# jperezrua/mfas

Measured on AMD Instinct MI355X. Metric: candidate-archs trained/sec (NTU inner loop), higher is better.
Workload: dtype f32

## Files before the change

### mfas_amd/csrc/mfas_hip.hip

```cpp
#include <hip/hip_runtime.h>
#include <hip/hip_fp16.h>
#pragma clang fp contract(off)
#include <stdint.h>
#include <stdio.h>
#include <string.h>
#include <math.h>
#include <cmath>
#include <algorithm>
#include <string>
#include <vector>
#include <thread>
#include <chrono>
#include <dlfcn.h>

#include "mfas_hip.h"

#include "common.hip.h"
#include "sweep.hip.h"
#include "chain.hip.h"

struct StepArgs {
    SweepArgs sa;
    ChainArgs ca;
    int32_t nchain, _pad;
    GatherArgs ga;
};

template <int MB, bool NT, int WPE, bool LEAN, int NS = 1>
__global__ void __launch_bounds__(STEP_THREADS, WPE) k_step(const StepArgs a) {
    extern __shared__ __attribute__((aligned(16))) float lds[];
    const int bid = (int)blockIdx.x;
    if (bid < a.nchain) {
        if constexpr (NS > 1) {
            const int Kp = a.nchain / NS, part = bid / Kp, c = bid - part * Kp;
            if (c < a.ca.ncand) chain_split<NS>(a.ca, chain_step_of(a.ca), c, part, lds);
        } else
        if constexpr (LEAN) { chain_lean<MB, 0, (WPE >= 4 ? 8 : 16)>(a.ca, chain_step_of(a.ca), bid, lds, lean_pre<MB>(a.ca, bid)); chain_lean_tail<MB, 0>(a.ca, chain_step_of(a.ca), bid, lds); }
        else chain_body<MB, false>(a.ca, chain_step_of(a.ca), bid, lds);
    }
    else if (bid < a.nchain + a.ga.nblocks) gather_body(a.ga, a.ga.cands[bid - a.nchain], a.sa.g, a.sa.tab, a.sa.order, (int)threadIdx.x);
    else if (bid < a.nchain + a.ga.nblocks + a.sa.ntap) sweep_tap_body<MB, NT, SweepU<MB, WPE>::v>(a.sa, bid - a.nchain - a.ga.nblocks, lds);
    else sweep_body<MB, NT, SweepU<MB, WPE>::v, false, !LEAN>(a.sa, sweep_step_of(a.sa), bid - a.nchain - a.ga.nblocks - a.sa.ntap, lds);
}

template <int MB, bool NT, int NS = 1>
__global__ void __launch_bounds__(STEP_THREADS, 4) k_step_same(const StepArgs a) {
    extern __shared__ __attribute__((aligned(16))) float lds[];
    const int bid = (int)blockIdx.x;
    if (bid < a.nchain) {
        if constexpr (NS > 1) {
            const int Kp = a.nchain / NS, part = bid / Kp, c = bid - part * Kp;
            if (c < a.ca.ncand) chain_split<NS>(a.ca, chain_step_of(a.ca), c, part, lds);
        } else chain_body<MB, false, true>(a.ca, chain_step_of(a.ca), bid, lds);
    } else sweep_body<MB, NT, SweepU<MB, 4>::v, true>(a.sa, sweep_step_of(a.sa), bid - a.nchain, lds);
}

template <int MB, bool LEAN>
__global__ void __launch_bounds__(STEP_THREADS, 2) k_chain(const ChainArgs a) {
    extern __shared__ __attribute__((aligned(16))) float lds[];
    if constexpr (LEAN) { chain_lean<MB>(a, chain_step_of(a), (int)blockIdx.x, lds, lean_pre<MB>(a, (int)blockIdx.x)); chain_lean_tail<MB, 0>(a, chain_step_of(a), (int)blockIdx.x, lds); }
    else chain_body<MB, true>(a, chain_step_of(a), (int)blockIdx.x, lds);
}

#include "wide.hip.h"
#include "persist.hip.h"
#include "eval.hip.h"
#include "pack.hip.h"
#include "surrogate.hip.h"

#include "builds.hip.h"
#include "plan.hip.h"
#ifdef MFAS_TEST_HOOKS
#include "plan_dump.hip.h"
#endif

struct LaunchRecord {
    struct Entry { BuildKey key; const void* fn; int64_t n; };
    std::vector<Entry> entries;
    void clear() { entries.clear(); }
    void count(const BuildKey& key, const void* fn) {
        for (Entry& e : entries) if (e.fn == fn) { ++e.n; return; }
        entries.push_back(Entry{key, fn, 1});
    }
    std::string describe() const {
        std::vector<std::string> items;
        for (const Entry& e : entries) items.push_back(e.key.name() + ":" + std::to_string(e.n));
        std::sort(items.begin(), items.end());
        std::string out;
        for (const std::string& s : items) out += (out.empty() ? "" : " ") + s;
        return out;
    }
};

struct mfas_population {
    mfas_hyper hp;
    Tuning tune;
    int K = 0, device = 0, n_cus = 0;
    int chunk_cols_req = 0;
    hipStream_t stream = nullptr;
    LayoutPlan plan;
    float* plane = nullptr;
    float* wt = nullptr;
    float* stepbuf = nullptr;
    float* best = nullptr;
    CandDev* d_cands = nullptr;
    SegDesc* d_descs = nullptr;
    struct GroupDev { SegDesc* d_descs = nullptr; TapDesc* d_taps = nullptr; };
    std::vector<GroupDev> groups;
    DevStats* d_stats = nullptr;
    int32_t* d_status = nullptr;
    uint32_t* d_seeds = nullptr;
    long long* d_corr = nullptr;
    float* d_posw = nullptr;
    int stats_cap = 0;
    bool profiling = false;
    int prof_every = 16;
    std::vector<hipEvent_t> ev;
    int64_t prof_launches = 0;
    double prof_ms = 0.0, bytes_per_launch = 0.0, prof_bytes = 0.0;
    LaunchRecord launched;
    double best_threshold = 0.0;
    struct Progress {
        std::vector<int64_t> done, nb;
        std::vector<double> best_metric;
        std::vector<int32_t> keeps_best;
        void reset(int K, double threshold) { done.assign(K, 0); nb.assign(K, 0); best_metric.assign(K, threshold); keeps_best.assign(K, 0); }
    } prog;
    float* d_move = nullptr;
    int64_t move_cap = 0;
    uint32_t* d_red_cnt = nullptr;
    char* d_gather = nullptr;
    size_t gather_cap = 0;
    uint32_t* d_cellflag = nullptr;
    float* d_xch = nullptr;
    SegDesc* d_pdescs = nullptr;
    int fell_back = 0;
    uint32_t* d_sync = nullptr;
    int32_t* d_need = nullptr;
    int32_t* d_role = nullptr;
    float* d_scal = nullptr;
    size_t scal_cap = 0;
    unsigned long long* d_trace = nullptr;
    char* d_vote = nullptr;
    size_t vote_cap = 0;
};

namespace {
struct Roctx {
    int (*push)(const char*) = nullptr;
    int (*pop)() = nullptr;
    Roctx() {
        if (getenv("MFAS_NO_ROCTX")) return;
        void* h = dlopen("librocprofiler-sdk-roctx.so", RTLD_LAZY | RTLD_LOCAL);
        if (!h) h = dlopen("librocprofiler-sdk-roctx.so.1", RTLD_LAZY | RTLD_LOCAL);
        if (!h) h = dlopen("libroctx64.so", RTLD_LAZY | RTLD_LOCAL);
        if (!h) return;
        push = reinterpret_cast<int (*)(const char*)>(dlsym(h, "roctxRangePushA"));
        pop = reinterpret_cast<int (*)()>(dlsym(h, "roctxRangePop"));
        if (!push || !pop) { push = nullptr; pop = nullptr; }
    }
};
Roctx& roctx() { static Roctx r; return r; }
struct RangeGuard {
    bool on;
    explicit RangeGuard(const std::string& name) : on(roctx().push != nullptr) { if (on) roctx().push(name.c_str()); }
    ~RangeGuard() { if (on) roctx().pop(); }
};
}
extern "C" int mfas_range_push(const char* name) { if (name && roctx().push) roctx().push(name); return MFAS_OK; }
extern "C" int mfas_range_pop(void) { if (roctx().pop) roctx().pop(); return MFAS_OK; }

extern "C" const char* mfas_last_error(void) { return g_err.c_str(); }
extern "C" int mfas_version(void) { return 200; }
#ifndef MFAS_SRC_DIGEST
#define MFAS_SRC_DIGEST "unknown"
#endif
extern "C" const char* mfas_source_digest(void) { return "mfas-src-digest:" MFAS_SRC_DIGEST; }

template <typename KT>
static hipError_t set_lds(KT kernel, size_t bytes) {
    return hipFuncSetAttribute(reinterpret_cast<const void*>(kernel), hipFuncAttributeMaxDynamicSharedMemorySize, (int)bytes);
}

static_assert(BUILDS_NTR == PERSIST_NTR && BUILDS_NTR16 == PERSIST_NTR16 && BUILDS_DT_BF16 == MFAS_DT_BF16, "builds.hip.h restates these");
typedef void (*StepKernel)(const StepArgs);
typedef void (*ChainKernel)(const ChainArgs);
typedef void (*PresidentKernel)(const PersistArgs, const int);
typedef hipError_t (*EvalLaunch)(mfas_population*, const EvalArgs&, int, hipStream_t);

template <typename KT>
struct Build { BuildKey key; KT fn = nullptr; };
typedef Build<StepKernel> StepBuild;
typedef Build<ChainKernel> ChainBuild;
typedef Build<PresidentKernel> PresidentBuild;
typedef Build<EvalLaunch> EvalBuild;

template <int MBE, int NRBW, int MSP, bool XB, bool B3>
static hipError_t launch_eval_t(mfas_population* p, const EvalArgs& a, int ncand, hipStream_t st);

template <int MB, bool NT, int WPE, bool LEAN, int NS> static StepBuild step_of() { return {step_key_of(MB, NT, WPE, LEAN, NS), k_step<MB, NT, WPE, LEAN, NS>}; }
template <int MB, bool NT, int NS> static StepBuild same_of() { return {same_key_of(MB, NT, NS), k_step_same<MB, NT, NS>}; }
template <bool NT> static StepBuild wide_sweep_of() { return {sweep_wide_key_of(NT), k_sweep_wide<NT>}; }
template <int MB, bool LEAN> static ChainBuild chain_of() { return {chain_key_of(MB, LEAN), k_chain<MB, LEAN>}; }
template <int MB, int NTR, bool X16, int NU, int PLAIN> static PresidentBuild president_of() { return {president_key_of(MB, NTR, X16, NU, PLAIN), k_president<MB, NTR, X16, NU, PLAIN>}; }
template <int MBE, int NRBW, int MSP, bool XB, bool B3> static EvalBuild eval_of() { return {eval_key_of(MBE, NRBW, MSP, XB, B3), launch_eval_t<MBE, NRBW, MSP, XB, B3>}; }

template <typename KT, size_t N>
static Build<KT> find_build(const Build<KT> (&rows)[N], const BuildKey& key) {
    for (const Build<KT>& r : rows) if (r.key == key) return r;
    return Build<KT>();
}

static StepBuild step_build(const BuildKey& key) {
#define STEP_(...) step_of<__VA_ARGS__>(),
#define SAME_(...) same_of<__VA_ARGS__>(),
#define WIDE_(...) wide_sweep_of<__VA_ARGS__>(),
    static const StepBuild rows[] = {BUILDS_SAME_ROWS(SAME_) BUILDS_STEP_ROWS(STEP_) BUILDS_SWEEP_WIDE_ROWS(WIDE_)};
#undef STEP_
#undef SAME_
#undef WIDE_
    return find_build(rows, key);
}

static ChainBuild chain_build(const BuildKey& key) {
#define CHAIN_(...) chain_of<__VA_ARGS__>(),
    static const ChainBuild rows[] = {BUILDS_CHAIN_ROWS(CHAIN_) {chain_wide_key_of(), k_chain_wide}};
#undef CHAIN_
    return find_build(rows, key);
}

static PresidentBuild president_build(const BuildKey& key) {
#define PRES_(...) president_of<__VA_ARGS__>(),
    static const PresidentBuild rows[] = {BUILDS_PRESIDENT_ROWS(PRES_)};
#undef PRES_
    return find_build(rows, key);
}

static EvalBuild eval_build(const BuildKey& key) {
#define EVAL_(...) eval_of<__VA_ARGS__>(),
    static const EvalBuild rows[] = {BUILDS_EVAL_ROWS(EVAL_)};
#undef EVAL_
    return find_build(rows, key);
}

template <typename... A>
static void launch(void (*kernel)(A...), unsigned grid, size_t lds, hipStream_t stream, A... args) {
    void* argv[] = {const_cast<void*>(static_cast<const void*>(&args))...};
    (void)hipLaunchKernel(reinterpret_cast<const void*>(kernel), dim3(grid), dim3(STEP_THREADS), argv, lds, stream);
}

template <typename... A>
static void launch_build(mfas_population* p, const Build<void (*)(A...)>& b, unsigned grid, size_t lds, hipStream_t stream, A... args) {
    if (b.fn) p->launched.count(b.key, reinterpret_cast<const void*>(b.fn));
    launch(b.fn, grid, lds, stream, args...);
}

static hipError_t set_lds_all(const LayoutPlan& pl) {
    hipError_t e = hipSuccess;
    auto set = [&e](auto kernel, size_t bytes) { if (kernel && e == hipSuccess) e = set_lds(kernel, bytes); };
    for (const BuildKey& key : plan_keys(plan_facts(pl)))
        switch (key.family) {
            case F_STEP: set(step_build(key).fn, key.arg[4] > 1 ? pl.lds_split : pl.lds_step); break;
            case F_STEP_SAME: set(step_build(key).fn, key.arg[2] > 1 ? pl.lds_split : pl.lds_step); break;
            case F_SWEEP_WIDE: set(step_build(key).fn, pl.lds_step); break;
            case F_CHAIN: case F_CHAIN_WIDE: set(chain_build(key).fn, pl.lds_chain); break;
            case F_PRESIDENT: set(president_build(key).fn, pl.lds_president); break;
            default: break;
        }
    return e;
}

static int device_cus(int device) {
    int ncu = 0;
    if (hipDeviceGetAttribute(&ncu, hipDeviceAttributeMultiprocessorCount, device) != hipSuccess || ncu <= 0) ncu = 256;
    return ncu;
}

template <typename T>
static hipError_t upload(T** dst, const std::vector<T>& v) {
    if (v.empty()) return hipSuccess;
    hipError_t e = hipMalloc(dst, sizeof(T) * v.size());
    return e != hipSuccess ? e : hipMemcpy(*dst, v.data(), sizeof(T) * v.size(), hipMemcpyHostToDevice);
}

static int create_impl(const mfas_hyper* hp, const int32_t* confs, const int32_t* n_cells,
                       const uint32_t* drop_seeds, int32_t K, int32_t device, void* hip_stream,
                       int32_t chunk_cols, mfas_population** out, const bool allow_persist, const Tuning* inherit = nullptr) {
    if (!out) return fail(MFAS_EINVAL, "null argument or K <= 0");
    if (int vrc = validate_inputs(hp, confs, n_cells, K)) return vrc;
    hipError_t e = hipSetDevice(device);
    if (e != hipSuccess) return fail(MFAS_EHIP, std::string("hipSetDevice: ") + hipGetErrorString(e));
    mfas_population* p = new (std::nothrow) mfas_population();
    if (!p) return fail(MFAS_ENOMEM, "host alloc");
    p->hp = *hp;
    p->tune = inherit ? *inherit : tuning_from_env();
    p->K = K;
    p->device = device;
    p->stream = reinterpret_cast<hipStream_t>(hip_stream);
    p->chunk_cols_req = chunk_cols;
    p->n_cus = device_cus(device);
    p->prog.reset(K, 0.0);
    if (int prc = plan_layout(hp, confs, n_cells, drop_seeds, K, chunk_cols, p->n_cus, allow_persist, p->tune, p->plan)) { delete p; return prc; }
    const LayoutPlan& pl = p->plan;
    if (!pl.fits_lds) { delete p; return fail(MFAS_EINVAL, "geometry does not fit the 160 KiB LDS (R / batchsize too large)"); }
    p->bytes_per_launch = pl.bytes_per_launch;

#define CREATE_CHK(x)                                                                              \
    do {                                                                                           \
        hipError_t e_ = (x);                                                                       \
        if (e_ != hipSuccess) {                                                                    \
            std::string m_ = std::string(#x) + ": " + hipGetErrorString(e_);                       \
            mfas_population_destroy(p);                                                            \
            return fail(e_ == hipErrorOutOfMemory ? MFAS_ENOMEM : MFAS_EHIP, m_);                  \
        }                                                                                          \
    } while (0)
    const size_t wt_floats = (size_t)std::max<int64_t>(pl.wt_size, 64);
    CREATE_CHK(hipMalloc(&p->plane, sizeof(float) * 3 * (size_t)pl.plane_stride));
    CREATE_CHK(hipMalloc(&p->wt, sizeof(float) * wt_floats));
    CREATE_CHK(hipMalloc(&p->stepbuf, sizeof(float) * (size_t)pl.step_total));
    CREATE_CHK(hipMalloc(&p->d_status, sizeof(int32_t) * (K + 256)));
    CREATE_CHK(hipMemset(p->d_status, 0, sizeof(int32_t) * (K + 256)));
    CREATE_CHK(hipMalloc(&p->d_seeds, sizeof(uint32_t) * K));
    CREATE_CHK(hipMalloc(&p->d_corr, sizeof(long long)));
    CREATE_CHK(upload(&p->d_posw, std::vector<float>(pl.g.Cp, 1.0f)));
    CREATE_CHK(upload(&p->d_cands, pl.cands));
    CREATE_CHK(upload(&p->d_descs, pl.descs));
    p->groups.resize(pl.groups.size());
    for (size_t gi = 0; gi < pl.groups.size(); ++gi) {
        CREATE_CHK(upload(&p->groups[gi].d_descs, pl.groups[gi].descs));
        CREATE_CHK(upload(&p->groups[gi].d_taps, pl.groups[gi].taps));
    }
    if (pl.red_in_sweep) {
        CREATE_CHK(hipMalloc(&p->d_red_cnt, sizeof(uint32_t) * K * MFAS_MAX_CELLS));
        CREATE_CHK(hipMemset(p->d_red_cnt, 0, sizeof(uint32_t) * K * MFAS_MAX_CELLS));
    }
    if (pl.same_group) CREATE_CHK(hipMalloc(&p->d_cellflag, sizeof(uint32_t) * K * CELLFLAG_STRIDE));
    if (pl.chain_split) CREATE_CHK(hipMalloc(&p->d_xch, sizeof(float) * (size_t)K * XCH_CAND_FLOATS));
    CREATE_CHK(hipMemsetAsync(p->plane, 0, sizeof(float) * 3 * (size_t)pl.plane_stride, p->stream));
    CREATE_CHK(hipMemsetAsync(p->wt, 0, sizeof(float) * wt_floats, p->stream));
    CREATE_CHK(hipMemsetAsync(p->stepbuf, 0, sizeof(float) * (size_t)pl.step_total, p->stream));
    CREATE_CHK(set_lds_all(pl));
    if (pl.persist) {
        CREATE_CHK(upload(&p->d_pdescs, pl.pdescs));
        CREATE_CHK(upload(&p->d_need, pl.need));
        CREATE_CHK(upload(&p->d_role, pl.role));
// ... 297 lines not shown
```

### mfas_amd/csrc/sweep.hip.h

```cpp
#pragma once
#include "launches.hip.h"
template <int MB, bool NT, int SWEEP_U, bool COH = false, bool DBL = false>
__device__ __forceinline__ void tile_run(float* Wp, float* Mp, float* Vp, const int rb, const int nkb, const int kb0,
                                         const int kbs, const float* xt, const int ST, const float* xn, const int SN,
                                         const float (&dyf)[MB * 4], const float gsc, const AdamC& ac, const bool upd,
                                         const bool fwd, f32x4 (&yacc)[MB], float* T, const int tstride_rb,
                                         const int lane, const int nj, const bool store = true, const float* xp = nullptr,
                                         const float* dyp = nullptr, const float* dyc = nullptr, const int SDp = 0,
                                         const float ss_p = 0.f, const float bc2s_p = 1.f) {
    static_assert(!(DBL && COH), "the same-group launch defers nothing");
    const int l15 = lane & 15, lg = lane >> 4;
    const float a_ss = ac.ss, a_bc2s = ac.bc2s, a_w1 = ac.w1, a_b2 = ac.b2, a_w2 = ac.w2, a_eps = ac.eps, a_wd = ac.wd;
    for (int kbb = kb0; kbb < nkb; kbb += SWEEP_U * kbs) {
        f32x4 w4[SWEEP_U], m4[SWEEP_U], v4[SWEEP_U];
#pragma unroll
        for (int u = 0; u < SWEEP_U; ++u) {
            const int kb = kbb + u * kbs;
            if (kb < nkb) {
                const int64_t off = ((int64_t)rb * nkb + kb) * 256 + lane * 4;
                w4[u] = NT ? __builtin_nontemporal_load(reinterpret_cast<const f32x4*>(Wp + off))
                           : *reinterpret_cast<const f32x4*>(Wp + off);
                if (upd) {
                    m4[u] = NT ? __builtin_nontemporal_load(reinterpret_cast<const f32x4*>(Mp + off))
                               : *reinterpret_cast<const f32x4*>(Mp + off);
                    v4[u] = NT ? __builtin_nontemporal_load(reinterpret_cast<const f32x4*>(Vp + off))
                               : *reinterpret_cast<const f32x4*>(Vp + off);
                }
            }
        }
#pragma unroll
        for (int u = 0; u < SWEEP_U; ++u) {
            const int kb = kbb + u * kbs;
            if (kb < nkb) {
                const int64_t off = ((int64_t)rb * nkb + kb) * 256 + lane * 4;
                if (upd) {
                    int dq = lg * SDp + rb * 16 + l15;
                    if constexpr (DBL) asm volatile("" : "+v"(dq));
                    if constexpr (DBL) {
                        f32x4 accp = {0.f, 0.f, 0.f, 0.f};
                        DW_BATCH_LOOP(MB, nj, accp = MFMA16(xp[(4 * j + lg) * ST + kb * 16 + l15], dyp[dq + 4 * j * SDp], accp))
                        f32x4 w = w4[u], m = m4[u], v = v4[u];
                        adam4(w, m, v, accp * gsc, ss_p, bc2s_p, a_w1, a_b2, a_w2, a_eps, a_wd);
                        w4[u] = w; m4[u] = m; v4[u] = v;
                        __builtin_amdgcn_sched_barrier(0);
                    }
                    f32x4 acc = {0.f, 0.f, 0.f, 0.f};
                    if constexpr (DBL) { DW_BATCH_LOOP(MB, nj, acc = MFMA16(xt[(4 * j + lg) * ST + kb * 16 + l15], dyc[dq + 4 * j * SDp], acc)) }
                    else { DW_BATCH_LOOP(MB, (COH ? MB * 4 : nj), acc = MFMA16(xt[(4 * j + lg) * ST + kb * 16 + l15], dyf[j], acc)) }
                    { f32x4 w = w4[u], m = m4[u], v = v4[u];
                      adam4(w, m, v, acc * gsc, a_ss, a_bc2s, a_w1, a_b2, a_w2, a_eps, a_wd);
                      w4[u] = w; m4[u] = m; v4[u] = v; }
                    if (!COH && !DBL && !store) {
                    } else if (NT) {
                        __builtin_nontemporal_store(w4[u], reinterpret_cast<f32x4*>(Wp + off));
                        __builtin_nontemporal_store(m4[u], reinterpret_cast<f32x4*>(Mp + off));
                        __builtin_nontemporal_store(v4[u], reinterpret_cast<f32x4*>(Vp + off));
                    } else {
                        *reinterpret_cast<f32x4*>(Wp + off) = w4[u];
                        *reinterpret_cast<f32x4*>(Mp + off) = m4[u];
                        *reinterpret_cast<f32x4*>(Vp + off) = v4[u];
                    }
                    if (T) {
                        float* Tt = T + ((int64_t)kb * tstride_rb + rb) * 256;
                        const int base = (((l15 >> 2) * 16 + 4 * lg) << 2) + (l15 & 3);
#pragma unroll
                        for (int q = 0; q < 4; ++q) Tt[base + 4 * q] = w4[u][q];
                    }
                }
                if (fwd) {
#pragma unroll
                    for (int mb = 0; mb < MB; ++mb) {
                        const f32x4 x4 = *reinterpret_cast<const f32x4*>(xn + (mb * 16 + l15) * SN + kb * 16 + 4 * lg);
#pragma unroll
                        for (int q = 0; q < 4; ++q) yacc[mb] = MFMA16(x4[q], w4[u][q], yacc[mb]);
                    }
                }
            }
        }
    }
}

#define STEP_NW 8
#define STEP_THREADS (STEP_NW * 64)

struct SweepArgs {
    const SegDesc* desc;
    const TapDesc* tdesc;
    int32_t ntap, _padt;
    const CandDev* cands;
    float* plane;
    int64_t plane_stride;
    float* wt;
    float* stepbuf;
    mfas_table tab;
    const int32_t* order;
    int64_t pos_t, pos_n;
    int32_t base_t, base_n, nvalid_t, nvalid_n;
    int32_t do_update, do_forward;
    AdamC ac;
    Geo g;
    uint32_t* red_cnt;
    const uint32_t* cellflag;
    uint32_t flag_target;
    int32_t* flag_status;
    const char* gather;
    int64_t g_cand_stride, g_par_stride;
    int32_t g_par_t, g_par_n;
    int32_t mode, g_par_p;
    int64_t pos_p, sb_dy_prev;
    int32_t base_p, nvalid_p;
    float ss_p, bc2s_p;
};

__device__ __forceinline__ int64_t gather_tap_off(const Geo& g, const int kind, const int tap, const int eb) {
    int64_t o = 0;
#pragma unroll
    for (int u = 0; u < MFAS_MAX_TAPS; ++u) {
        if (kind == KIND_V || u < tap) o += g.sw[u];
        if (kind == KIND_V && u < tap) o += g.vw[u];
    }
    return o * g.Bp * eb;
}

struct GatherArgs {
    const CandDev* cands;
    char* buf;
    int64_t cand_stride, par_stride;
    int64_t pos[2];
    int32_t base[2], nvalid[2], par[2];
    int32_t nsets, nblocks;
};

__device__ __forceinline__ void gather_body(const GatherArgs& ga, const CandDev& cd, const Geo& g, const mfas_table& tab,
                                            const int32_t* order, const int tid) {
    const int eb = tab.dtype == MFAS_DT_F32 ? 4 : 2;
    const int32_t* ordp = cand_order(order, g, cd.gidx);
    uint32_t used = 0;
    for (int i = 0; i < cd.L; ++i) used |= (1u << cd.conf[i][0]) | (1u << (MFAS_MAX_TAPS + cd.conf[i][1]));
#pragma unroll
    for (int s = 0; s < 2; ++s) {
        if (s >= ga.nsets) break;
        char* dst0 = ga.buf + (int64_t)cd.gidx * ga.cand_stride + (int64_t)ga.par[s] * ga.par_stride;
        for (int kt = 0; kt < 2 * MFAS_MAX_TAPS; ++kt) {
            if (!((used >> kt) & 1u)) continue;
            const int kind = kt < MFAS_MAX_TAPS ? KIND_S : KIND_V, tap = kt & (MFAS_MAX_TAPS - 1);
            const int w = kind == KIND_S ? g.sw[tap] : g.vw[tap];
            const char* src0 = reinterpret_cast<const char*>(kind == KIND_S ? tab.s[tap] : tab.v[tap]);
            char* dst = dst0 + gather_tap_off(g, kind, tap, eb);
            const int vpr = (w * eb) >> 4, nvec = ga.nvalid[s] * vpr;
            for (int e0 = tid; e0 < nvec; e0 += 4 * STEP_THREADS) {
                u32x4 v[4];
#pragma unroll
                for (int u = 0; u < 4; ++u) {
                    const int e = e0 + u * STEP_THREADS;
                    if (e < nvec) {
                        const int b = e / vpr, c = e - b * vpr;
                        const int64_t row = ordp ? (int64_t)ordp[ga.pos[s] + b] : (int64_t)(ga.base[s] + b);
                        v[u] = *reinterpret_cast<const u32x4*>(src0 + (row * w) * eb + ((int64_t)c << 4));
                    }
                }
#pragma unroll
                for (int u = 0; u < 4; ++u) {
                    const int e = e0 + u * STEP_THREADS;
                    if (e < nvec) {
                        const int b = e / vpr, c = e - b * vpr;
                        *reinterpret_cast<u32x4*>(dst + ((int64_t)b * w) * eb + ((int64_t)c << 4)) = v[u];
                    }
                }
            }
        }
    }
}

struct SweepStep {
    int64_t pos_t, pos_n;
    int32_t base_t, base_n, nvalid_t, nvalid_n;
    int32_t upd, fwd;
    float ss, bc2s;
};
__device__ __forceinline__ SweepStep sweep_step_of(const SweepArgs& a) {
    SweepStep s;
    s.pos_t = a.pos_t; s.pos_n = a.pos_n; s.base_t = a.base_t; s.base_n = a.base_n;
    s.nvalid_t = a.nvalid_t; s.nvalid_n = a.nvalid_n; s.upd = a.do_update; s.fwd = a.do_forward;
    s.ss = a.ac.ss; s.bc2s = a.ac.bc2s;
    return s;
}


#ifdef MFAS_CHAIN_TIMING
#define SW_UNIT_STAMP(k) do { if (COH && a.cellflag && a.flag_target == 16u && threadIdx.x == 0 && d.cell == 0 && d.kind == KIND_S && d.k0 == 0 && d.cand == 0) a.flag_status[64 + 29 + (k)] = (int32_t)wall_clock64(); } while (0)
#define SW_END_STAMP() do { if (COH && a.cellflag && a.flag_target == 16u && threadIdx.x == 0) { atomicMax(reinterpret_cast<uint32_t*>(&a.flag_status[64 + 27]), (uint32_t)wall_clock64()); \
        atomicMax(reinterpret_cast<uint32_t*>(&a.flag_status[128 + d.cell * 4 + d.kind]), (uint32_t)wall_clock64()); } } while (0)
#else
#define SW_END_STAMP() do { } while (0)
#define SW_UNIT_STAMP(k) do { } while (0)
#endif
template <int MB, bool NT, int U, bool COH = false, bool DEFER = !COH>
__device__ __forceinline__ void sweep_body(const SweepArgs& a, const SweepStep& st, const int bid, float* lds) {
    const SegDesc d = a.desc[bid];
    const CandDev& cd = a.cands[d.cand];
    const int tid = threadIdx.x, lane = tid & 63, wave = tid >> 6;
    const int l15 = lane & 15, lg = lane >> 4;
    constexpr int Bp = MB * 16;
    const int cc = d.cc, rows_p = d.rows_p, nrb = rows_p >> 4, nkb = cc >> 4;
    const int ST = cc + 16;
    const int SN = cc + 4;
    const int SD = rows_p + 16;
    float* xt = lds;
    float* xn = xt + Bp * ST;
    float* dyl = xn + Bp * SN;
    const bool feat = d.kind <= KIND_V;
    const bool upd = st.upd != 0;
    const bool fwd = (st.fwd != 0) && feat;
    if (!upd && !fwd) return;
    float* wred = dyl + Bp * SD;
    const bool split_k = nrb < STEP_NW;
    const int mode = (DEFER && feat && upd) ? a.mode : LAUNCH_PLAIN;
    const bool dbl = mode == LAUNCH_DOUBLE;
    float* xp = wred + (split_k ? (nrb - 1) * STEP_NW * MB * 256 : 0);
    float* dyp = xp + Bp * ST;
    const int64_t sbo = cd.step_off;
    const bool red = a.red_cnt != nullptr;

    if (!COH && a.gather && feat) {
        const char* gb = a.gather + (int64_t)cd.gidx * a.g_cand_stride + gather_tap_off(a.g, d.kind, d.tap, a.tab.dtype == MFAS_DT_F32 ? 4 : 2);
        if (dbl) stage_table(xp, ST, gb + (int64_t)a.g_par_p * a.g_par_stride, a.tab.dtype, d.width, d.k0, cc, nullptr, 0, 0, a.nvalid_p, Bp, tid, STEP_THREADS);
        if (upd) stage_table(xt, ST, gb + (int64_t)a.g_par_t * a.g_par_stride, a.tab.dtype, d.width, d.k0, cc, nullptr, 0, 0, st.nvalid_t, Bp, tid, STEP_THREADS);
        if (fwd) stage_table(xn, SN, gb + (int64_t)a.g_par_n * a.g_par_stride, a.tab.dtype, d.width, d.k0, cc, nullptr, 0, 0, st.nvalid_n, Bp, tid, STEP_THREADS);
    } else {
    if (upd && feat) {
        const void* tp = d.kind == KIND_S ? a.tab.s[d.tap] : a.tab.v[d.tap];
        if (dbl) stage_table(xp, ST, tp, a.tab.dtype, d.width, d.k0, cc, cand_order(a.order, a.g, cd.gidx), a.pos_p, a.base_p, a.nvalid_p, Bp, tid, STEP_THREADS);
        stage_table(xt, ST, tp, a.tab.dtype, d.width, d.k0, cc, cand_order(a.order, a.g, cd.gidx), st.pos_t, st.base_t, st.nvalid_t, Bp, tid, STEP_THREADS);
    }
    if (fwd) {
        const void* tp = d.kind == KIND_S ? a.tab.s[d.tap] : a.tab.v[d.tap];
        stage_table(xn, SN, tp, a.tab.dtype, d.width, d.k0, cc, cand_order(a.order, a.g, cd.gidx), st.pos_n, st.base_n, st.nvalid_n, Bp, tid, STEP_THREADS);
    }
    }
    if constexpr (COH) {
        if (upd && a.cellflag) {
            __shared__ int s_go;
            if (tid == 0) {
                const int slot = d.kind == KIND_HEAD ? cd.L - 1 : (d.kind == KIND_OUT ? d.cell - 1 : d.cell);
                const uint32_t* f = a.cellflag + (size_t)cd.gidx * CELLFLAG_STRIDE + slot;
                uint32_t spins = 0;
                int go = 1;
                while (ld_u32_relaxed(f) < a.flag_target) {
                    __builtin_amdgcn_s_sleep(2);
                    if (++spins > CELLFLAG_SPIN_LIMIT) { go = 0; atomicMax(&a.flag_status[cd.gidx], 2); break; }
                }
                s_go = go;
#ifdef MFAS_CHAIN_TIMING
                if (a.flag_target == 16u && slot == 0 && d.kind <= KIND_V) atomicMin(reinterpret_cast<uint32_t*>(&a.flag_status[64 + 28]), (uint32_t)wall_clock64());
#endif
            }
            __syncthreads();
            if (!s_go) return;
            SW_UNIT_STAMP(0);
        }
    }
    if (upd) {
        if (!feat) {
            const int xcell = d.kind == KIND_OUT ? d.cell - 1 : cd.L - 1;
            stage_f32<COH>(xt, ST, a.stepbuf, sbo + a.g.sb_xo + (int64_t)xcell * Bp * a.g.Rp + d.k0, a.g.Rp, cc, Bp, tid, STEP_THREADS);
        }
        const int64_t dsrc = d.kind == KIND_HEAD ? sbo + a.g.sb_dlog : sbo + a.g.sb_dy + (int64_t)d.cell * Bp * a.g.Rp;
        stage_f32<COH>(dyl, SD, a.stepbuf, dsrc + d.rb0 * 16, d.seg_nrb * 16, rows_p, Bp, tid, STEP_THREADS);
        if (dbl) stage_f32<false>(dyp, SD, a.stepbuf, sbo + a.sb_dy_prev + (int64_t)d.cell * Bp * a.g.Rp + d.rb0 * 16, d.seg_nrb * 16, rows_p, Bp, tid, STEP_THREADS);
    }
    __syncthreads();
    SW_UNIT_STAMP(1);

    float* Wp = a.plane + d.w_off;
    float* Mp = Wp + a.plane_stride;
    float* Vp = Mp + a.plane_stride;
    const AdamC ac = adam_consts(a.ac, upd ? st.ss : 0.f, upd ? st.bc2s : 1.f);
    float gsc = 1.0f;
    if (a.g.alphas && feat && upd) gsc = ldc1<COH>(a.stepbuf + sbo + a.g.sb_gsc + d.cell * 2 + d.kind);

    const int rb0 = split_k ? 0 : wave, rbs = split_k ? 1 : STEP_NW;
    const int kb0 = split_k ? wave : 0, kbs = split_k ? STEP_NW : 1;
    const int64_t part = sbo + a.g.sb_part + (((int64_t)(cd.part_cell_off[d.cell] + d.part_idx) * d.seg_nrb * MB) << 8) +
                         (((int64_t)d.rb0 * MB) << 8);

    for (int rb = rb0; rb < nrb; rb += rbs) {
        float dyf[MB * 4];
        f32x4 yacc[MB];
#pragma unroll
        for (int mb = 0; mb < MB; ++mb) yacc[mb] = (f32x4){0.f, 0.f, 0.f, 0.f};
        float* Tt = d.wt_off >= 0 ? a.wt + d.wt_off + ((int64_t)(d.k0 >> 4) * d.seg_nrb + d.rb0) * 256 : nullptr;
        bool plain_walk = true;
        if constexpr (DEFER) {
            if (dbl) {
                plain_walk = false;
                tile_run<MB, NT, (U > 1 ? U / 2 : 1), false, true>(Wp, Mp, Vp, rb, nkb, kb0, kbs, xt, ST, xn, SN, dyf, gsc, ac, upd, fwd, yacc, Tt, d.seg_nrb,
                                                                    lane, (a.g.B + 3) >> 2, true, xp, dyp, dyl, SD, a.ss_p, a.bc2s_p);
                if (split_k && fwd && rb == nrb - 1) __syncthreads();
            }
        }
        if (plain_walk) {
#pragma unroll
            for (int j = 0; j < MB * 4; ++j) dyf[j] = upd ? dyl[(4 * j + lg) * SD + rb * 16 + l15] : 0.f;
            tile_run<MB, NT, U, COH>(Wp, Mp, Vp, rb, nkb, kb0, kbs, xt, ST, xn, SN, dyf, gsc, ac, upd, fwd, yacc, Tt, d.seg_nrb, lane,
                                     (a.g.B + 3) >> 2, mode != LAUNCH_VIRTUAL);
        }
        if (fwd) {
#pragma unroll
            for (int mb = 0; mb < MB; ++mb) {
                if (split_k)
                    *reinterpret_cast<f32x4*>(wred + (((rb * STEP_NW + wave) * MB + mb) << 8) + lane * 4) = yacc[mb];
                else if (red) stc4<true>(a.stepbuf, part + ((rb * MB + mb) << 8) + lane * 4, yacc[mb]);
                else
                    stc4<COH>(a.stepbuf, part + ((rb * MB + mb) << 8) + lane * 4, yacc[mb]);
            }
        }
    }
    SW_UNIT_STAMP(2);
    if (!fwd) { SW_END_STAMP(); return; }
    if (split_k) {
        __syncthreads();
        for (int e = tid; e < nrb * MB * 64; e += STEP_THREADS) {
            const int slot = e >> 6, ln = e & 63;
            const int srb = slot / MB, smb = slot - srb * MB;
            f32x4 s = *reinterpret_cast<const f32x4*>(wred + (((srb * STEP_NW) * MB + smb) << 8) + ln * 4);
#pragma unroll
            for (int w = 1; w < STEP_NW; ++w)
                s += *reinterpret_cast<const f32x4*>(wred + (((srb * STEP_NW + w) * MB + smb) << 8) + ln * 4);
            if (red) stc4<true>(a.stepbuf, part + (slot << 8) + ln * 4, s);
            else stc4<COH>(a.stepbuf, part + (slot << 8) + ln * 4, s);
        }
    }
    if (!red) { SW_END_STAMP(); return; }
    asm volatile("s_waitcnt vmcnt(0)" ::: "memory");
    __syncthreads();
    SW_UNIT_STAMP(3);
    int* flagw = reinterpret_cast<int*>(lds);
    const int ns_c = cd.nch_s[d.cell], nch_c = ns_c + cd.nch_v[d.cell];
    if (tid == 0) {
        uint32_t* cnt = a.red_cnt + d.cand * MFAS_MAX_CELLS + d.cell;
        const uint32_t old = __hip_atomic_fetch_add(cnt, 1u, __ATOMIC_RELAXED, __HIP_MEMORY_SCOPE_AGENT);
        const int last = old == (uint32_t)(nch_c - 1);
        if (last) __hip_atomic_store(cnt, 0u, __ATOMIC_RELAXED, __HIP_MEMORY_SCOPE_AGENT);
        flagw[0] = last;
    }
    __syncthreads();
    SW_UNIT_STAMP(4);
    if (!flagw[0]) { SW_END_STAMP(); return; }
    {
        const int snrb = d.seg_nrb;
        const int per_cell = snrb * MB * 64;
        const int64_t part0 = sbo + a.g.sb_part + (((int64_t)cd.part_cell_off[d.cell] * snrb * MB) << 8);
        const int64_t yf0 = sbo + a.g.sb_yf + (int64_t)d.cell * per_cell * 4;
        const int64_t vplane = (int64_t)MFAS_MAX_CELLS * snrb * MB * 256;
        for (int it = tid; it < per_cell; it += STEP_THREADS) {
            f32x4 accS = {0.f, 0.f, 0.f, 0.f}, accV = {0.f, 0.f, 0.f, 0.f};
            constexpr int PB = 8;
            for (int ch0 = 0; ch0 < nch_c; ch0 += PB) {
                f32x4 p8[PB];
#pragma unroll
                for (int u = 0; u < PB; ++u)
                    if (ch0 + u < nch_c) p8[u] = ldc4<true>(a.stepbuf, part0 + (((int64_t)(ch0 + u) * snrb * MB) << 8) + it * 4);
#pragma unroll
                for (int u = 0; u < PB; ++u)
                    if (ch0 + u < nch_c) {
                        if (ch0 + u < ns_c) accS += p8[u]; else accV += p8[u];
                    }
            }
            if (a.g.alphas) {
                *reinterpret_cast<f32x4*>(a.stepbuf + yf0 + it * 4) = accS;
                *reinterpret_cast<f32x4*>(a.stepbuf + yf0 + vplane + it * 4) = accV;
            } else {
                *reinterpret_cast<f32x4*>(a.stepbuf + yf0 + it * 4) = accS + accV;
            }
        }
    }
    SW_END_STAMP();
}

template <int MB, bool NT, int U>
__device__ __forceinline__ void sweep_tap_body(const SweepArgs& a, const int bid, float* lds) {
    const TapDesc& d = a.tdesc[bid];
    const int tid = threadIdx.x, lane = tid & 63, wave = tid >> 6;
    const int l15 = lane & 15, lg = lane >> 4;
    constexpr int Bp = MB * 16;
    const int cc = d.cc, rows_p = d.rows_p, nrb = rows_p >> 4, nkb = cc >> 4;
    const int ST = cc + 16, SN = cc + 4;
    float* xt = lds;
    float* xn = xt + Bp * ST;
    const bool upd = a.do_update != 0;
    const bool fwd = a.do_forward != 0;
    if (!upd && !fwd) return;
    const void* tp = d.kind == KIND_S ? a.tab.s[d.tap] : a.tab.v[d.tap];
    if (upd) stage_table(xt, ST, tp, a.tab.dtype, d.width, d.k0, cc, a.order, a.pos_t, a.base_t, a.nvalid_t, Bp, tid, STEP_THREADS);
    if (fwd) stage_table(xn, SN, tp, a.tab.dtype, d.width, d.k0, cc, a.order, a.pos_n, a.base_n, a.nvalid_n, Bp, tid, STEP_THREADS);
    __syncthreads();
    const int item = wave / nrb, rb = wave - item * nrb;
    if (item >= d.nitems) return;
    const CandDev& cd = a.cands[d.cand[item]];
    float* sb = a.stepbuf + cd.step_off;
    const int cell = d.cell[item];
    float dyf[MB * 4];
#pragma unroll
    for (int j = 0; j < MB * 4; ++j) dyf[j] = 0.f;
    if (upd) {
        const float* dsrc = sb + a.g.sb_dy + (int64_t)cell * Bp * a.g.Rp;
#pragma unroll
        for (int j = 0; j < MB * 4; ++j) dyf[j] = dsrc[(4 * j + lg) * rows_p + rb * 16 + l15];
    }
    float gsc = 1.0f;
    if (a.g.alphas && upd) gsc = sb[a.g.sb_gsc + cell * 2 + d.kind];
    float* Wp = a.plane + d.w_off[item];
    float* Mp = Wp + a.plane_stride;
    float* Vp = Mp + a.plane_stride;
    const AdamC ac = adam_consts(a.ac, a.ac.ss, a.ac.bc2s);
    f32x4 yacc[MB];
#pragma unroll
    for (int mb = 0; mb < MB; ++mb) yacc[mb] = (f32x4){0.f, 0.f, 0.f, 0.f};
    tile_run<MB, NT, U>(Wp, Mp, Vp, rb, nkb, 0, 1, xt, ST, xn, SN, dyf, gsc, ac, upd, fwd, yacc, nullptr, nrb, lane, (a.g.B + 3) >> 2);
    if (fwd) {
        float* part = sb + a.g.sb_part + (((int64_t)(cd.part_cell_off[cell] + d.part_idx[item]) * nrb * MB) << 8);
#pragma unroll
        for (int mb = 0; mb < MB; ++mb)
            *reinterpret_cast<f32x4*>(part + ((rb * MB + mb) << 8) + lane * 4) = yacc[mb];
    }
}
```

Before: 37.29.

## Add software-pipelined double-buffered sweep tile loop for MB=1, WPE=4 fused step

Factors the sweep tile body (load, dW MFMA plus Adam update, store, forward MFMA) into helpers. It adds a new tile_pipe path that double-buffers the W/M/V loads, issuing the next tile's loads before processing the current one, with sched barriers to keep that order. The path also makes wave and loop indices scalar via readfirstlane. It is enabled only for the k_step sweep when MB==1, WPE==4 and not LEAN, and only for feature segments doing both update and forward without a transposed copy. The aim is to hide global-memory latency in the optimizer sweep, at the cost of more registers and a second code path that must stay consistent with tile_run.

New measurement: 39.06, median of 6. +4.7%, better.

```diff
diff --git a/mfas_amd/csrc/mfas_hip.hip b/mfas_amd/csrc/mfas_hip.hip
--- a/mfas_amd/csrc/mfas_hip.hip
+++ b/mfas_amd/csrc/mfas_hip.hip
@@ -40,7 +40,7 @@
     }
     else if (bid < a.nchain + a.ga.nblocks) gather_body(a.ga, a.ga.cands[bid - a.nchain], a.sa.g, a.sa.tab, a.sa.order, (int)threadIdx.x);
     else if (bid < a.nchain + a.ga.nblocks + a.sa.ntap) sweep_tap_body<MB, NT, SweepU<MB, WPE>::v>(a.sa, bid - a.nchain - a.ga.nblocks, lds);
-    else sweep_body<MB, NT, SweepU<MB, WPE>::v, false, !LEAN>(a.sa, sweep_step_of(a.sa), bid - a.nchain - a.ga.nblocks - a.sa.ntap, lds);
+    else sweep_body<MB, NT, SweepU<MB, WPE>::v, false, !LEAN, SweepPipe<MB, WPE, LEAN>::v>(a.sa, sweep_step_of(a.sa), bid - a.nchain - a.ga.nblocks - a.sa.ntap, lds);
 }
 
 template <int MB, bool NT, int NS = 1>
diff --git a/mfas_amd/csrc/sweep.hip.h b/mfas_amd/csrc/sweep.hip.h
--- a/mfas_amd/csrc/sweep.hip.h
+++ b/mfas_amd/csrc/sweep.hip.h
@@ -1,5 +1,63 @@
 #pragma once
 #include "launches.hip.h"
+template <bool NT>
+__device__ __forceinline__ f32x4 tile_ld(const float* p) {
+    return NT ? __builtin_nontemporal_load(reinterpret_cast<const f32x4*>(p)) : *reinterpret_cast<const f32x4*>(p);
+}
+template <int MB, bool COH>
+__device__ __forceinline__ void tile_update(f32x4& w, f32x4& m, f32x4& v, const float* xt, const int ST, const int kb,
+                                            const float (&dyf)[MB * 4], const int nj, const int l15, const int lg, const float gsc,
+                                            const float ss, const float bc2s, const float w1, const float b2, const float w2,
+                                            const float eps, const float wd) {
+    f32x4 acc = {0.f, 0.f, 0.f, 0.f};
+    DW_BATCH_LOOP(MB, (COH ? MB * 4 : nj), acc = MFMA16(xt[(4 * j + lg) * ST + kb * 16 + l15], dyf[j], acc))
+    adam4(w, m, v, acc * gsc, ss, bc2s, w1, b2, w2, eps, wd);
+}
+template <int MB>
+__device__ __forceinline__ void tile_update_lds(f32x4& w, f32x4& m, f32x4& v, const float* x, const int ST, const int kb,
+                                                const float* dy, const int dq, const int SD, const int nj, const int l15, const int lg,
+                                                const float gsc, const float ss, const float bc2s, const float w1, const float b2,
+                                                const float w2, const float eps, const float wd) {
+    f32x4 acc = {0.f, 0.f, 0.f, 0.f};
+    DW_BATCH_LOOP(MB, nj, acc = MFMA16(x[(4 * j + lg) * ST + kb * 16 + l15], dy[dq + 4 * j * SD], acc))
+    adam4(w, m, v, acc * gsc, ss, bc2s, w1, b2, w2, eps, wd);
+}
+template <int MB>
+__device__ __forceinline__ void tile_replay(f32x4& w, f32x4& m, f32x4& v, const float* xp, const int ST, const int kb, const float* dyp,
+                                            const int dq, const int SD, const int nj, const int l15, const int lg, const float gsc,
+                                            const float ss_p, const float bc2s_p, const float w1, const float b2, const float w2,
+                                            const float eps, const float wd) {
+    tile_update_lds<MB>(w, m, v, xp, ST, kb, dyp, dq, SD, nj, l15, lg, gsc, ss_p, bc2s_p, w1, b2, w2, eps, wd);
+    __builtin_amdgcn_sched_barrier(0);
+}
+template <bool NT>
+__device__ __forceinline__ void tile_store(const f32x4 w, const f32x4 m, const f32x4 v, float* Wp, float* Mp, float* Vp, const int64_t off) {
+    if (NT) {
+        __builtin_nontemporal_store(w, reinterpret_cast<f32x4*>(Wp + off));
+        __builtin_nontemporal_store(m, reinterpret_cast<f32x4*>(Mp + off));
+        __builtin_nontemporal_store(v, reinterpret_cast<f32x4*>(Vp + off));
+    } else {
+        *reinterpret_cast<f32x4*>(Wp + off) = w;
+        *reinterpret_cast<f32x4*>(Mp + off) = m;
+        *reinterpret_cast<f32x4*>(Vp + off) = v;
+    }
+}
+__device__ __forceinline__ void tile_store_t(const f32x4 w, float* T, const int kb, const int tstride_rb, const int rb, const int l15, const int lg) {
+    float* Tt = T + ((int64_t)kb * tstride_rb + rb) * 256;
+    const int base = (((l15 >> 2) * 16 + 4 * lg) << 2) + (l15 & 3);
+#pragma unroll
+    for (int q = 0; q < 4; ++q) Tt[base + 4 * q] = w[q];
+}
+template <int MB>
+__device__ __forceinline__ void tile_forward(f32x4 (&yacc)[MB], const float* xn, const int SN, const int kb, const int l15, const int lg, const f32x4 w) {
+#pragma unroll
+    for (int mb = 0; mb < MB; ++mb) {
+        const f32x4 x4 = *reinterpret_cast<const f32x4*>(xn + (mb * 16 + l15) * SN + kb * 16 + 4 * lg);
+#pragma unroll
+        for (int q = 0; q < 4; ++q) yacc[mb] = MFMA16(x4[q], w[q], yacc[mb]);
+    }
+}
+
 template <int MB, bool NT, int SWEEP_U, bool COH = false, bool DBL = false>
 __device__ __forceinline__ void tile_run(float* Wp, float* Mp, float* Vp, const int rb, const int nkb, const int kb0,
                                          const int kbs, const float* xt, const int ST, const float* xn, const int SN,
@@ -18,13 +76,10 @@
             const int kb = kbb + u * kbs;
             if (kb < nkb) {
                 const int64_t off = ((int64_t)rb * nkb + kb) * 256 + lane * 4;
-                w4[u] = NT ? __builtin_nontemporal_load(reinterpret_cast<const f32x4*>(Wp + off))
-                           : *reinterpret_cast<const f32x4*>(Wp + off);
+                w4[u] = tile_ld<NT>(Wp + off);
                 if (upd) {
-                    m4[u] = NT ? __builtin_nontemporal_load(reinterpret_cast<const f32x4*>(Mp + off))
-                               : *reinterpret_cast<const f32x4*>(Mp + off);
-                    v4[u] = NT ? __builtin_nontemporal_load(reinterpret_cast<const f32x4*>(Vp + off))
-                               : *reinterpret_cast<const f32x4*>(Vp + off);
+                    m4[u] = tile_ld<NT>(Mp + off);
+                    v4[u] = tile_ld<NT>(Vp + off);
                 }
             }
         }
@@ -34,49 +89,86 @@
             if (kb < nkb) {
                 const int64_t off = ((int64_t)rb * nkb + kb) * 256 + lane * 4;
                 if (upd) {
-                    int dq = lg * SDp + rb * 16 + l15;
-                    if constexpr (DBL) asm volatile("" : "+v"(dq));
                     if constexpr (DBL) {
-                        f32x4 accp = {0.f, 0.f, 0.f, 0.f};
-                        DW_BATCH_LOOP(MB, nj, accp = MFMA16(xp[(4 * j + lg) * ST + kb * 16 + l15], dyp[dq + 4 * j * SDp], accp))
-                        f32x4 w = w4[u], m = m4[u], v = v4[u];
-                        adam4(w, m, v, accp * gsc, ss_p, bc2s_p, a_w1, a_b2, a_w2, a_eps, a_wd);
-                        w4[u] = w; m4[u] = m; v4[u] = v;
-                        __builtin_amdgcn_sched_barrier(0);
+                        int dq = lg * SDp + rb * 16 + l15;
+                        asm volatile("" : "+v"(dq));
+                        tile_replay<MB>(w4[u], m4[u], v4[u], xp, ST, kb, dyp, dq, SDp, nj, l15, lg, gsc, ss_p, bc2s_p, a_w1, a_b2, a_w2, a_eps, a_wd);
+                        tile_update_lds<MB>(w4[u], m4[u], v4[u], xt, ST, kb, dyc, dq, SDp, nj, l15, lg, gsc, a_ss, a_bc2s, a_w1, a_b2, a_w2, a_eps, a_wd);
+                    } else {
+                        tile_update<MB, COH>(w4[u], m4[u], v4[u], xt, ST, kb, dyf, nj, l15, lg, gsc, a_ss, a_bc2s, a_w1, a_b2, a_w2, a_eps, a_wd);
                     }
-                    f32x4 acc = {0.f, 0.f, 0.f, 0.f};
-                    if constexpr (DBL) { DW_BATCH_LOOP(MB, nj, acc = MFMA16(xt[(4 * j + lg) * ST + kb * 16 + l15], dyc[dq + 4 * j * SDp], acc)) }
-                    else { DW_BATCH_LOOP(MB, (COH ? MB * 4 : nj), acc = MFMA16(xt[(4 * j + lg) * ST + kb * 16 + l15], dyf[j], acc)) }
-                    { f32x4 w = w4[u], m = m4[u], v = v4[u];
-                      adam4(w, m, v, acc * gsc, a_ss, a_bc2s, a_w1, a_b2, a_w2, a_eps, a_wd);
-                      w4[u] = w; m4[u] = m; v4[u] = v; }
                     if (!COH && !DBL && !store) {
-                    } else if (NT) {
-                        __builtin_nontemporal_store(w4[u], reinterpret_cast<f32x4*>(Wp + off));
-                        __builtin_nontemporal_store(m4[u], reinterpret_cast<f32x4*>(Mp + off));
-                        __builtin_nontemporal_store(v4[u], reinterpret_cast<f32x4*>(Vp + off));
                     } else {
-                        *reinterpret_cast<f32x4*>(Wp + off) = w4[u];
-                        *reinterpret_cast<f32x4*>(Mp + off) = m4[u];
-                        *reinterpret_cast<f32x4*>(Vp + off) = v4[u];
+                        tile_store<NT>(w4[u], m4[u], v4[u], Wp, Mp, Vp, off);
                     }
-                    if (T) {
-                        float* Tt = T + ((int64_t)kb * tstride_rb + rb) * 256;
-                        const int base = (((l15 >> 2) * 16 + 4 * lg) << 2) + (l15 & 3);
-#pragma unroll
-                        for (int q = 0; q < 4; ++q) Tt[base + 4 * q] = w4[u][q];
-                    }
+                    if (T) tile_store_t(w4[u], T, kb, tstride_rb, rb, l15, lg);
                 }
-                if (fwd) {
-#pragma unroll
-                    for (int mb = 0; mb < MB; ++mb) {
-                        const f32x4 x4 = *reinterpret_cast<const f32x4*>(xn + (mb * 16 + l15) * SN + kb * 16 + 4 * lg);
-#pragma unroll
-                        for (int q = 0; q < 4; ++q) yacc[mb] = MFMA16(x4[q], w4[u][q], yacc[mb]);
-                    }
-                }
-            }
-        }
+                if (fwd) tile_forward<MB>(yacc, xn, SN, kb, l15, lg, w4[u]);
+            }
+        }
+    }
+}
+
+template <int MB, bool NT, int PASS>
+__device__ __forceinline__ void tile_pipe(float* Wp, float* Mp, float* Vp, const int rb_, const int nkb_, const int kb0_, const int kbs_,
+                                          const float* xt, const int ST, const float* xn, const int SN, const float (&dyf)[MB * 4],
+                                          const float gsc, const AdamC& ac, f32x4 (&yacc)[MB], const int lane, const int nj,
+                                          const float* xp = nullptr, const float* dyp = nullptr, const float* dyc = nullptr,
+                                          const int SDp = 0, const float ss_p = 0.f, const float bc2s_p = 1.f) {
+    static_assert(PASS == LAUNCH_PLAIN || PASS == LAUNCH_DOUBLE, "a virtual pass keeps tile_run (sweep_body)");
+    const int rb = __builtin_amdgcn_readfirstlane(rb_), nkb = __builtin_amdgcn_readfirstlane(nkb_);
+    const int kb0 = __builtin_amdgcn_readfirstlane(kb0_), kbs = __builtin_amdgcn_readfirstlane(kbs_);
+    if (kb0 >= nkb) return;
+    const float a_ss = ac.ss, a_bc2s = ac.bc2s, a_w1 = ac.w1, a_b2 = ac.b2, a_w2 = ac.w2, a_eps = ac.eps, a_wd = ac.wd;
+    const int n = kbs == 1 ? nkb - kb0 : (nkb - kb0 + kbs - 1) / kbs;
+    const int64_t off0 = (int64_t)rb * nkb * 256 + lane * 4;
+    auto request = [&](f32x4& w, f32x4& m, f32x4& v, const int kb) __attribute__((always_inline)) {
+        const int64_t off = off0 + (int64_t)kb * 256;
+        w = tile_ld<NT>(Wp + off);
+        m = tile_ld<NT>(Mp + off);
+        v = tile_ld<NT>(Vp + off);
+        __builtin_amdgcn_sched_barrier(0);
+    };
+    auto work = [&](f32x4& w, f32x4& m, f32x4& v, const int kb) __attribute__((always_inline)) {
+        int l15 = lane & 15, lg = lane >> 4;
+        asm volatile("" : "+v"(l15), "+v"(lg));
+        if constexpr (PASS == LAUNCH_DOUBLE) {
+            int dq = lg * SDp + rb * 16 + l15;
+            asm volatile("" : "+v"(dq));
+            tile_replay<MB>(w, m, v, xp, ST, kb, dyp, dq, SDp, nj, l15, lg, gsc, ss_p, bc2s_p, a_w1, a_b2, a_w2, a_eps, a_wd);
+            tile_update_lds<MB>(w, m, v, xt, ST, kb, dyc, dq, SDp, nj, l15, lg, gsc, a_ss, a_bc2s, a_w1, a_b2, a_w2, a_eps, a_wd);
+        } else {
+            tile_update<MB, false>(w, m, v, xt, ST, kb, dyf, nj, l15, lg, gsc, a_ss, a_bc2s, a_w1, a_b2, a_w2, a_eps, a_wd);
+        }
+        tile_store<NT>(w, m, v, Wp, Mp, Vp, off0 + (int64_t)kb * 256);
+        tile_forward<MB>(yacc, xn, SN, kb, l15, lg, w);
+        __builtin_amdgcn_sched_barrier(0);
+    };
+    f32x4 wA, mA, vA, wB, mB, vB;
+    int kb = kb0;
+    if (n == 1) {
+        request(wA, mA, vA, kb);
+        work(wA, mA, vA, kb);
+        return;
+    }
+    request(wA, mA, vA, kb);
+    request(wB, mB, vB, kb + kbs);
+    work(wA, mA, vA, kb);
+    int left = n - 1;
+    while (left >= 3) {
+        request(wA, mA, vA, kb + 2 * kbs);
+        work(wB, mB, vB, kb + kbs);
+        request(wB, mB, vB, kb + 3 * kbs);
+        work(wA, mA, vA, kb + 2 * kbs);
+        kb += 2 * kbs;
+        left -= 2;
+    }
+    if (left == 2) {
+        request(wA, mA, vA, kb + 2 * kbs);
+        work(wB, mB, vB, kb + kbs);
+        work(wA, mA, vA, kb + 2 * kbs);
+    } else {
+        work(wB, mB, vB, kb + kbs);
     }
 }
 
@@ -195,11 +287,13 @@
 #define SW_END_STAMP() do { } while (0)
 #define SW_UNIT_STAMP(k) do { } while (0)
 #endif
-template <int MB, bool NT, int U, bool COH = false, bool DEFER = !COH>
+template <int MB, int WPE, bool LEAN> struct SweepPipe { static constexpr bool v = MB == 1 && WPE == 4 && !LEAN; };
+template <int MB, bool NT, int U, bool COH = false, bool DEFER = !COH, bool PIPE = false>
 __device__ __forceinline__ void sweep_body(const SweepArgs& a, const SweepStep& st, const int bid, float* lds) {
     const SegDesc d = a.desc[bid];
     const CandDev& cd = a.cands[d.cand];
-    const int tid = threadIdx.x, lane = tid & 63, wave = tid >> 6;
+    const int tid = threadIdx.x, lane = tid & 63;
+    const int wave = PIPE ? __builtin_amdgcn_readfirstlane(tid >> 6) : tid >> 6;
     const int l15 = lane & 15, lg = lane >> 4;
     constexpr int Bp = MB * 16;
     const int cc = d.cc, rows_p = d.rows_p, nrb = rows_p >> 4, nkb = cc >> 4;
@@ -291,8 +385,25 @@
         for (int mb = 0; mb < MB; ++mb) yacc[mb] = (f32x4){0.f, 0.f, 0.f, 0.f};
         float* Tt = d.wt_off >= 0 ? a.wt + d.wt_off + ((int64_t)(d.k0 >> 4) * d.seg_nrb + d.rb0) * 256 : nullptr;
         bool plain_walk = true;
+        bool piped = false;
+        if constexpr (PIPE && !COH) {
+            if (feat && upd && fwd && !Tt && mode != LAUNCH_VIRTUAL) {
+                piped = true;
+                plain_walk = false;
+                const int nj = (a.g.B + 3) >> 2;
+                if (DEFER && dbl) {
+                    tile_pipe<MB, NT, LAUNCH_DOUBLE>(Wp, Mp, Vp, rb, nkb, kb0, kbs, xt, ST, xn, SN, dyf, gsc, ac, yacc, lane, nj, xp, dyp, dyl, SD,
+                                                   a.ss_p, a.bc2s_p);
+                    if (split_k && rb == nrb - 1) __syncthreads();
+                } else {
+#pragma unroll
+                    for (int j = 0; j < MB * 4; ++j) dyf[j] = dyl[(4 * j + lg) * SD + rb * 16 + l15];
+                    tile_pipe<MB, NT, LAUNCH_PLAIN>(Wp, Mp, Vp, rb, nkb, kb0, kbs, xt, ST, xn, SN, dyf, gsc, ac, yacc, lane, nj);
+                }
+            }
+        }
         if constexpr (DEFER) {
-            if (dbl) {
+            if (dbl && !piped) {
                 plain_walk = false;
                 tile_run<MB, NT, (U > 1 ? U / 2 : 1), false, true>(Wp, Mp, Vp, rb, nkb, kb0, kbs, xt, ST, xn, SN, dyf, gsc, ac, upd, fwd, yacc, Tt, d.seg_nrb,
                                                                     lane, (a.g.B + 3) >> 2, true, xp, dyp, dyl, SD, a.ss_p, a.bc2s_p);
```
